# maybeLx/MVSFormerPlusPlus

Hardware: NVIDIA H100
Metric: depth-maps/sec (hot path: FMT + 4-stage cascade) (higher is better)
Workload: dtype f32

## Files before the change

### include/mvsf_b200.h

```cpp
#ifndef MVSF_B200_H
#define MVSF_B200_H

#include <stddef.h>
#include <stdint.h>

#ifdef __cplusplus
extern "C" {
#endif

typedef void* mvsf_stream_t;

enum mvsf_status {
  MVSF_OK = 0,
  MVSF_ERR_INVALID = -1,
  MVSF_ERR_CUDA = -2,
  MVSF_ERR_WORKSPACE = -3
};

const char* mvsf_last_error(void);
int mvsf_abi_version(void);
long long mvsf_launch_count(int reset);
int mvsf_ktimer_enable(int on);
int mvsf_ktimer_read(const char* name, double* ms, long long* launches);

// ... 1 lines not shown
int mvsf_nhwc_to_nchw(const float* src, float* dst, int N, int C, int HW, mvsf_stream_t stream);

int mvsf_compose_geometry(const float* proj, int V, float* homs, float* kinv_ref, mvsf_stream_t stream);

int mvsf_homography_from_proj(const float* src_proj, const float* ref_proj, int B, float* homs, mvsf_stream_t stream);

int mvsf_init_inverse_range(const float* depth_values, int Dn, float* out, int D, int H, int W, mvsf_stream_t stream);
int mvsf_schedule_inverse_range(const float* prev_depth, const float* prev_hypo, int Dp, float split_itv, float* out,
                                int D, int H, int W, mvsf_stream_t stream);
int mvsf_position3d(const float* kinv_ref, const float* depth, const float* depth_values, int Dn, float* stats,
                    int compute_minmax, float* pos, int D, int H, int W, mvsf_stream_t stream);

int mvsf_homo_warp(const float* src_nhwc, const float* hom, const float* depth, float* warped, uint8_t* mask, int C,
                   int D, int H, int W, mvsf_stream_t stream);

int mvsf_warp_corr_set_tile_path(int mode);
int mvsf_warp_corr_set_max_window_miss(int permille);
int mvsf_warp_corr_last_selection(int* used_pipeline, int* miss_permille);

int mvsf_set_prefer_shared_carveout(int on);

int mvsf_warp_corr_plan(int C, int G, int D, int H, int W, int V, size_t spill_budget_bytes);

int mvsf_warp_corr_entropy(const float* feat, const float* homs, const float* depth, float* entropy, int V, int C,
                           int G, int D, int H, int W, mvsf_stream_t stream);
int mvsf_vis_cnn_set_precision(int x_lo);

int mvsf_vis_cnn(const float* entropy, const float* wts, float* vis, int N, int H, int W, mvsf_stream_t stream);
int mvsf_warp_corr_aggregate(const float* feat, const float* homs, const float* depth, const float* vis,
                             float* volume, int V, int C, int G, int D, int H, int W, mvsf_stream_t stream);
int mvsf_warp_corr_entropy_store(const float* feat, const float* homs, const float* depth, float* entropy, float* corr,
                                 int V, int C, int G, int D, int H, int W, mvsf_stream_t stream);
int mvsf_corr_aggregate(const float* corr, const float* vis, float* volume, int V, int G, int D, int H, int W,
                        mvsf_stream_t stream);

int mvsf_costreg_unet_workspace_bytes(int kind, int C, int D, int H, int W, size_t* bytes);
int mvsf_costreg_unet_tc_bytes(size_t* bytes);
int mvsf_costreg_unet_pack_tc(int kind, const float* wts, void* wts_tc, size_t wts_tc_bytes, mvsf_stream_t stream);
int mvsf_costreg_unet_forward(int kind, const float* volume, const float* wts, const void* wts_tc, float* logits,
                              void* workspace, size_t workspace_bytes, int C, int D, int H, int W, mvsf_stream_t stream);
int mvsf_conv3d_tc_layer(int mode, int sd, const float* in, const float* w32, const float* skip, float* out,
                         void* workspace, size_t workspace_bytes, int cin, int cout, int ID, int IH, int IW,
                         mvsf_stream_t stream);

int mvsf_costreg_tr_workspace_bytes(int C, int D, int H, int W, size_t* bytes);
int mvsf_costreg_tr_forward(float* volume, const float* pos, const float* wts, const void* wts16, size_t n_wts,
                            float* logits, void* workspace, size_t workspace_bytes, int C, int D, int H, int W,
                            int layers, float softmax_scale, mvsf_stream_t stream);
int mvsf_split_weights_f16(const float* wts, void* out16, size_t n, mvsf_stream_t stream);

int mvsf_attention_forward(const float* qkv, float* out, void* workspace, size_t workspace_bytes, int N,
                           float softmax_scale, mvsf_stream_t stream);

int mvsf_linear_tc_forward(const float* A, const float* W, const float* bias, float* C, void* workspace,
                           size_t workspace_bytes, int M, int N, int K, int gelu, mvsf_stream_t stream);
int mvsf_linear_tc_epilogue(int epi, const float* A, int lda, const float* W, const float* bias, const float* res,
                            int ldres, const float* gamma, const float* ln_w, const float* ln_b, float ln_eps,
                            int elu_cols, float* C, int ldc, float* Cpre, int ldcpre, void* C2, int ldc2,
                            void* workspace, size_t workspace_bytes, int M, int N, int K, mvsf_stream_t stream);
int mvsf_linear_tc_streamed_epilogue(int epi, const float* A, int lda, const float* W, const float* bias,
                                     const float* res, int ldres, const float* gamma, int elu_cols, float* C, int ldc,
                                     void* C2, int ldc2, void* workspace, size_t workspace_bytes, int M, int N, int K,
                                     mvsf_stream_t stream);

int mvsf_softargmax(const float* logits, const float* depth_hypo, float tmp, float* prob, float* depth, float* conf,
                    int D, int H, int W, mvsf_stream_t stream);
int mvsf_conf_accumulate(const float* conf, int h, int w, float* acc, int H, int W, float scale, int init,
                         mvsf_stream_t stream);

int mvsf_fmt_workspace_bytes(int V, int H1, int W1, size_t* bytes);
int mvsf_fmt_forward(const float* f1, const float* f2, const float* f3, const float* f4, const float* pe,
                     const float* wts, const void* wts16, size_t n_wts, float* o1, float* o2, float* o3, float* o4,
                     void* workspace, size_t workspace_bytes, int V, int H1, int W1, mvsf_stream_t stream);

int mvsf_fpn_encoder_workspace_bytes(int N, int H, int W, size_t* bytes);
int mvsf_fpn_encoder_forward(const float* x, const float* wts, const void* wts_tc, float* c01, float* c11, float* c21,
                             float* c31, void* workspace, size_t workspace_bytes, int N, int H, int W, mvsf_stream_t stream);
int mvsf_fpn_encoder_vit_forward(const float* x, const float* vit_feat, int V, const float* wts, const void* wts_tc,
                                 float* c01, float* c11, float* c21, float* c31, void* workspace, size_t workspace_bytes,
                                 int N, int H, int W, mvsf_stream_t stream);
int mvsf_fpn_decoder_workspace_bytes(int N, int H, int W, size_t* bytes);
int mvsf_fpn_decoder_forward(const float* c01, const float* c11, const float* c21, const float* c31, const float* wts,
                             const void* wts_tc, float* o0, float* o1, float* o2, float* o3, void* workspace,
                             size_t workspace_bytes, int N, int H, int W, mvsf_stream_t stream);
int mvsf_fpn_tc_bytes(int part, size_t* bytes);
int mvsf_fpn_pack_tc(int part, const float* wts, void* wts_tc, size_t wts_tc_bytes, mvsf_stream_t stream);

int mvsf_vit_decoder_workspace_bytes(int B, int V, int h, int w, size_t* bytes);
int mvsf_vit_decoder_tc_bytes(size_t* bytes);
int mvsf_vit_decoder_pack_tc(const float* wts, void* wts_tc, size_t wts_tc_bytes, mvsf_stream_t stream);
int mvsf_vit_decoder_forward(const float* x0, const float* x1, const float* x2, const float* wts, const void* wts_tc,
                             float* out, void* workspace, size_t workspace_bytes, int B, int V, int h, int w,
                             mvsf_stream_t stream);

int mvsf_vit_workspace_bytes(int n, int gh, int gw, size_t* bytes);
int mvsf_vit_tc_bytes(size_t* bytes);
int mvsf_vit_pack_tc(const float* wts, void* wts_tc, size_t wts_tc_bytes, mvsf_stream_t stream);
int mvsf_vit_forward(const float* img, const float* pos, const float* wts, const void* wts_tc, float* out0, float* out1,
                     float* out2, void* workspace, size_t workspace_bytes, int n, int gh, int gw, mvsf_stream_t stream);
int mvsf_vit_forward_image(const float* img, int H, int W, const float* pos, const float* wts, const void* wts_tc,
                           float* out0, float* out1, float* out2, void* workspace, size_t workspace_bytes, int n, int gh,
                           int gw, mvsf_stream_t stream);
int mvsf_vit_attention_forward(const float* qkv, int ldq, float* out, int ldo, void* workspace, size_t workspace_bytes,
                               int n, int N, mvsf_stream_t stream);

#ifdef __cplusplus
// ... 4 lines not shown
```

### mvsformerplusplus_b200/_lib.py

```python
import ctypes
import os

_HERE = os.path.dirname(os.path.abspath(__file__))
LIB_PATH = os.environ.get("MVSF_LIB_PATH") or os.path.join(_HERE, "libmvsf_b200.so")
_lib = None

P, I, F, Z = ctypes.c_void_p, ctypes.c_int, ctypes.c_float, ctypes.c_size_t
SIGNATURES = {
    "mvsf_abi_version": ([], I),
    "mvsf_launch_count": ([I], ctypes.c_longlong),
    "mvsf_ktimer_enable": ([I], I),
    "mvsf_ktimer_read": ([ctypes.c_char_p, ctypes.POINTER(ctypes.c_double), ctypes.POINTER(ctypes.c_longlong)], I),
    "mvsf_nchw_to_nhwc": ([P, P, I, I, I, P], I),
    "mvsf_nhwc_to_nchw": ([P, P, I, I, I, P], I),
    "mvsf_compose_geometry": ([P, I, P, P, P], I),
    "mvsf_homography_from_proj": ([P, P, I, P, P], I),
    "mvsf_init_inverse_range": ([P, I, P, I, I, I, P], I),
    "mvsf_schedule_inverse_range": ([P, P, I, F, P, I, I, I, P], I),
    "mvsf_position3d": ([P, P, P, I, P, I, P, I, I, I, P], I),
    "mvsf_homo_warp": ([P, P, P, P, P, I, I, I, I, P], I),
    "mvsf_warp_corr_set_tile_path": ([I], I),
    "mvsf_warp_corr_set_max_window_miss": ([I], I),
    "mvsf_set_prefer_shared_carveout": ([I], I),
    "mvsf_warp_corr_last_selection": ([ctypes.POINTER(I), ctypes.POINTER(I)], I),
    "mvsf_warp_corr_plan": ([I, I, I, I, I, I, Z], I),
    "mvsf_warp_corr_entropy": ([P, P, P, P, I, I, I, I, I, I, P], I),
    "mvsf_vis_cnn_set_precision": ([I], I),
    "mvsf_vis_cnn": ([P, P, P, I, I, I, P], I),
    "mvsf_warp_corr_aggregate": ([P, P, P, P, P, I, I, I, I, I, I, P], I),
    "mvsf_warp_corr_entropy_store": ([P, P, P, P, P, I, I, I, I, I, I, P], I),
    "mvsf_corr_aggregate": ([P, P, P, I, I, I, I, I, P], I),
    "mvsf_costreg_unet_workspace_bytes": ([I, I, I, I, I, ctypes.POINTER(Z)], I),
    "mvsf_costreg_unet_tc_bytes": ([ctypes.POINTER(Z)], I),
    "mvsf_costreg_unet_pack_tc": ([I, P, P, Z, P], I),
    "mvsf_costreg_unet_forward": ([I, P, P, P, P, P, Z, I, I, I, I, P], I),
    "mvsf_conv3d_tc_layer": ([I, I, P, P, P, P, P, Z, I, I, I, I, I, P], I),
    "mvsf_costreg_tr_workspace_bytes": ([I, I, I, I, ctypes.POINTER(Z)], I),
    "mvsf_costreg_tr_forward": ([P, P, P, P, Z, P, P, Z, I, I, I, I, I, F, P], I),
    "mvsf_split_weights_f16": ([P, P, Z, P], I),
    "mvsf_attention_forward": ([P, P, P, Z, I, F, P], I),
    "mvsf_linear_tc_forward": ([P, P, P, P, P, Z, I, I, I, I, P], I),
    "mvsf_linear_tc_epilogue": ([I, P, I, P, P, P, I, P, P, P, F, I, P, I, P, I, P, I, P, Z, I, I, I, P], I),
    "mvsf_softargmax": ([P, P, F, P, P, P, I, I, I, P], I),
    "mvsf_conf_accumulate": ([P, I, I, P, I, I, F, I, P], I),
    "mvsf_fmt_workspace_bytes": ([I, I, I, ctypes.POINTER(Z)], I),
    "mvsf_fmt_forward": ([P] * 7 + [Z] + [P] * 5 + [Z, I, I, I, P], I),
    "mvsf_fpn_encoder_workspace_bytes": ([I, I, I, ctypes.POINTER(Z)], I),
    "mvsf_fpn_encoder_forward": ([P] * 8 + [Z, I, I, I, P], I),
    "mvsf_fpn_encoder_vit_forward": ([P, P, I] + [P] * 7 + [Z, I, I, I, P], I),
    "mvsf_fpn_decoder_workspace_bytes": ([I, I, I, ctypes.POINTER(Z)], I),
    "mvsf_fpn_decoder_forward": ([P] * 11 + [Z, I, I, I, P], I),
    "mvsf_fpn_tc_bytes": ([I, ctypes.POINTER(Z)], I),
    "mvsf_fpn_pack_tc": ([I, P, P, Z, P], I),
    "mvsf_linear_tc_streamed_epilogue": ([I, P, I, P, P, P, I, P, I, P, I, P, I, P, Z, I, I, I, P], I),
    "mvsf_vit_decoder_workspace_bytes": ([I, I, I, I, ctypes.POINTER(Z)], I),
    "mvsf_vit_decoder_tc_bytes": ([ctypes.POINTER(Z)], I),
    "mvsf_vit_decoder_pack_tc": ([P, P, Z, P], I),
    "mvsf_vit_decoder_forward": ([P] * 7 + [Z, I, I, I, I, P], I),
    "mvsf_vit_workspace_bytes": ([I, I, I, ctypes.POINTER(Z)], I),
    "mvsf_vit_tc_bytes": ([ctypes.POINTER(Z)], I),
    "mvsf_vit_pack_tc": ([P, P, Z, P], I),
    "mvsf_vit_forward": ([P] * 8 + [Z, I, I, I, P], I),
    "mvsf_vit_forward_image": ([P, I, I] + [P] * 7 + [Z, I, I, I, P], I),
    "mvsf_vit_attention_forward": ([P, I, P, I, P, Z, I, I, P], I),
}


def lib():
    global _lib
    if _lib is None:
        if not os.path.exists(LIB_PATH):
            raise RuntimeError(f"{LIB_PATH} is missing: build it with `python -m mvsformerplusplus_b200.build` "
                               "(the hot path has no CPU/PyTorch fallback)")
        L = ctypes.CDLL(LIB_PATH)
        L.mvsf_last_error.restype = ctypes.c_char_p
        L.mvsf_last_error.argtypes = []
        for name, (argt, rest) in SIGNATURES.items():
            fn = getattr(L, name)
            fn.argtypes = argt
            fn.restype = rest
        if os.environ.get("MVSF_VIS_XLO") in ("0", "1"):
            L.mvsf_vis_cnn_set_precision(int(os.environ["MVSF_VIS_XLO"]))
        if os.environ.get("MVSF_WARP_TILE", "1") in ("0", "2"):
            L.mvsf_warp_corr_set_tile_path(int(os.environ["MVSF_WARP_TILE"]))
        if os.environ.get("MVSF_PREFER_SHARED") in ("0", "1"):
            L.mvsf_set_prefer_shared_carveout(int(os.environ["MVSF_PREFER_SHARED"]))
        if os.environ.get("MVSF_WT_MAX_MISS"):
            L.mvsf_warp_corr_set_max_window_miss(int(os.environ["MVSF_WT_MAX_MISS"]))
        _lib = L
    return _lib


def check(rc, what):
    if rc != 0:
        msg = lib().mvsf_last_error().decode(errors="replace")
        raise RuntimeError(f"{what} failed (status {rc}): {msg}")


def launch_count(reset=False):
    return int(lib().mvsf_launch_count(1 if reset else 0))


class profile_calls:

    def __init__(self):
        self.records = []

    def __enter__(self):
        import torch
        L = lib()
        self._orig = {}
        for name in SIGNATURES:
            if name.endswith("_workspace_bytes") or name in ("mvsf_abi_version", "mvsf_launch_count", "mvsf_ktimer_enable",
                                                             "mvsf_ktimer_read", "mvsf_warp_corr_plan",
                                                             "mvsf_warp_corr_set_tile_path", "mvsf_warp_corr_set_max_window_miss", "mvsf_set_prefer_shared_carveout",
                                                             "mvsf_warp_corr_last_selection", "mvsf_vis_cnn_set_precision"):
                continue
            fn = getattr(L, name)
            self._orig[name] = fn

            def wrapped(*a, _fn=fn, _name=name):
                s, e = torch.cuda.Event(enable_timing=True), torch.cuda.Event(enable_timing=True)
                s.record()
                rc = _fn(*a)
                e.record()
                self.records.append((_name, s, e))
                return rc
            setattr(L, name, wrapped)
        return self

    def __exit__(self, *exc):
        L = lib()
        for name, fn in self._orig.items():
            setattr(L, name, fn)
        return False

    def summary(self):
        import torch
        torch.cuda.synchronize()
        out = {}
        for name, s, e in self.records:
            d = out.setdefault(name, {"ms": 0.0, "calls": 0})
            d["ms"] += s.elapsed_time(e)
            d["calls"] += 1
        return out


def ktimer_enable(on):
    check(lib().mvsf_ktimer_enable(1 if on else 0), "ktimer_enable")


def ktimer_read(name):
    ms, n = ctypes.c_double(0.0), ctypes.c_longlong(0)
    check(lib().mvsf_ktimer_read(name.encode(), ctypes.byref(ms), ctypes.byref(n)), "ktimer_read")
    return ms.value, n.value
```

### mvsformerplusplus_b200/csrc/attention_fa.cuh

```cuda
#pragma once
#include <cuda_fp16.h>

#include "linear_tc.cuh"
#include "softmax_attention.cuh"
#include "wgmma.cuh"

namespace mvsf {

__global__ void qkv_tile_kernel(const float* __restrict__ qkv, __half* __restrict__ tiled, int N, int ntiles, float qscale) {
  const int i = blockIdx.x * blockDim.x + threadIdx.x;
  const int total = ntiles * 128 * 3 * 4 * 2;
  if (i >= total) return;
  const int oct = i & 1, h = (i >> 1) & 3, which = (i >> 3) % 3, tok = i / 24;
  const size_t plane = (size_t)4 * ntiles * 2048;
  const int tile = tok >> 7, r = tok & 127;
  float v[8];
  if (tok < N) {
    const float4 a = ldg4(qkv + (size_t)tok * 192 + which * 64 + h * 16 + oct * 8);
    const float4 b = ldg4(qkv + (size_t)tok * 192 + which * 64 + h * 16 + oct * 8 + 4);
    v[0] = a.x; v[1] = a.y; v[2] = a.z; v[3] = a.w; v[4] = b.x; v[5] = b.y; v[6] = b.z; v[7] = b.w;
    if (which == 0) {
#pragma unroll
      for (int e = 0; e < 8; ++e) v[e] *= qscale;
    }
  } else {
#pragma unroll
    for (int e = 0; e < 8; ++e) v[e] = 0.f;
  }
  if (which < 2) {
    __half* ph = tiled + (size_t)(which * 2) * plane + ((size_t)h * ntiles + tile) * 2048;
    __half* pl = ph + plane;
    split_store8(ph + oct * 1024 + r * 8, pl + oct * 1024 + r * 8, v);
  } else {
    __half* pv = tiled + (size_t)4 * plane + ((size_t)h * ntiles + tile) * 5120;
    const int kc = r >> 3, e = r & 7;
#pragma unroll
    for (int d = 0; d < 8; ++d) {
      __half hi, lo;
      gmma::split_f16(v[d], hi, lo);
      pv[kc * 320 + (oct * 8 + d) * 8 + e] = lo;
      pv[kc * 320 + (16 + oct * 8 + d) * 8 + e] = hi;
    }
    if (oct == 0) {
      pv[kc * 320 + 32 * 8 + e] = __float2half_rn(1.0f);
    } else {
#pragma unroll
      for (int z = 33; z < 40; ++z) pv[kc * 320 + z * 8 + e] = __float2half_rn(0.f);
    }
  }
}

namespace fa {
using namespace gmma;
template <int NWG_>
struct Layout {
  static constexpr int NWG = NWG_, NKV = 3, REGS_PRODUCER = 32, REGS_CONSUMER = 160, HD = 16, NH = 4, O_REGS = 20;
  static constexpr uint32_t LBO_QK = 2048, LBO_Q = 1024, LBO_V = 640;
  static constexpr uint32_t K_TILE = 4096, Q_BLOCK = 4096, V_TILE = 16 * LBO_V;
  static constexpr uint32_t OFF_K = 0, OFF_V = OFF_K + NKV * 2 * K_TILE, OFF_Q = OFF_V + NKV * V_TILE,
                            OFF_BAR = OFF_Q + NWG * Q_BLOCK, SMEM = OFF_BAR + 8 + 32 * NKV;
  static constexpr int THREADS = 128 * (NWG + 1);

  const __half* tiled;
  const __half* base;
  size_t plane, head_tiles;

  struct QOperand { uint64_t hi, lo; };
  static __device__ __forceinline__ QOperand q_operand(uint32_t q) {
    return {make_desc(q, LBO_Q, 128), make_desc(q + Q_BLOCK / 2, LBO_Q, 128)};
  }
  static __device__ __forceinline__ void issue_scores(float (&S)[64], const QOperand& q, uint32_t kt) {
    const uint64_t k_hi = make_desc(kt, LBO_QK, 128), k_lo = make_desc(kt + K_TILE, LBO_QK, 128);
    mma_ss<128>(S, q.lo, k_hi, 0u);
    mma_ss<128>(S, q.hi, k_lo, 1u);
    mma_ss<128>(S, q.hi, k_hi, 1u);
    wg_commit();
  }
  static __device__ __forceinline__ void issue_pv(float (&O)[20], const uint32_t (&ph)[8][4], uint32_t vt) {
#pragma unroll
    for (int i = 0; i < 8; ++i) mma_rs_n40(O, ph[i], make_desc(vt + 2 * i * LBO_V, LBO_V, 128), i > 0 ? 1u : 0u);
    wg_commit();
  }
  static __device__ __forceinline__ void fold_tile(float (&o)[2][4], float (&l)[2], const float (&O)[20], const float (&corr)[2],
                                                   int lane) {
#pragma unroll
    for (int h = 0; h < 2; ++h) {
#pragma unroll
      for (int b = 0; b < 2; ++b)
#pragma unroll
        for (int e = 0; e < 2; ++e) o[h][2 * b + e] = fmaf(o[h][2 * b + e], corr[h], O[4 * b + 2 * h + e] + O[4 * (b + 2) + 2 * h + e]);
      const float lt = __shfl_sync(0xffffffffu, O[16 + 2 * h], lane & ~3);
      l[h] = fmaf(l[h], corr[h], lt);
    }
  }
  static __device__ __forceinline__ int q_blocks(int N, int ntiles) { return 2 * ntiles; }
  __device__ __forceinline__ void load_q(uint32_t dst, int b, uint32_t bar) const {
    for (int p = 0; p < 2; ++p)
      for (int kc = 0; kc < 2; ++kc)
        bulk_load(dst + p * (Q_BLOCK / 2) + kc * LBO_Q, base + p * plane + (size_t)(b >> 1) * 2048 + kc * 1024 + (b & 1) * 512,
                  LBO_Q, bar);
  }
  __device__ __forceinline__ const __half* k_tile(int t, int p) const { return base + (2 + p) * plane + (size_t)t * 2048; }
  __device__ __forceinline__ const __half* v_tile(int t) const { return tiled + 4 * plane + (head_tiles + t) * (V_TILE / 2); }
  __device__ __forceinline__ size_t row(int t) const { return (size_t)t; }
};
}

template <int NWG>
__global__ void __launch_bounds__(fa::Layout<NWG>::THREADS, 1)
attention_fa_kernel(const __half* __restrict__ tiled, float* __restrict__ out, __half* __restrict__ out2, int N, int ntiles) {
  const int head = blockIdx.y;
  const size_t head_tiles = (size_t)head * ntiles;
  const fa::Layout<NWG> lay{tiled, tiled + head_tiles * 2048, (size_t)4 * ntiles * 2048, head_tiles};
  attn::softmax_attention(lay, out, 64, out2, N, ntiles);
}

}
```

### mvsformerplusplus_b200/csrc/costreg_tr.cu

```cuda
#include <cuda_fp16.h>
#include <float.h>

#include "attention_fa.cuh"
#include "linear_tc.cuh"
#include "wgmma.cuh"

namespace mvsf {

constexpr int TR_PE = 0, TR_DOWN_W = 192, TR_DOWN_B = TR_DOWN_W + 64 * 256, TR_DOWN_LNW = TR_DOWN_B + 64,
              TR_DOWN_LNB = TR_DOWN_LNW + 64, TR_LAYER0 = TR_DOWN_LNB + 64;
constexpr int L_QKV = 0, L_PROJ_W = 192 * 64, L_PROJ_B = L_PROJ_W + 64 * 64, L_G1 = L_PROJ_B + 64, L_N1W = L_G1 + 64,
              L_N1B = L_N1W + 64, L_F1W = L_N1B + 64, L_F1B = L_F1W + 256 * 64, L_F2W = L_F1B + 256,
              L_F2B = L_F2W + 64 * 256, L_G2 = L_F2B + 64, L_N2W = L_G2 + 64, L_N2B = L_N2W + 64, TR_LAYER = L_N2B + 64;
constexpr int U_W = 0, U_B = 256 * 64, U_LNW = U_B + 256, U_LNB = U_LNW + 8, U_PW = U_LNB + 8, U_PB = U_PW + 8;

__global__ void pe3d_add_kernel(float* __restrict__ vol, const float* __restrict__ pos, const float* __restrict__ pe_w,
                                size_t nvox) {
  __shared__ float w[8 * 24];
  for (int i = threadIdx.x; i < 192; i += blockDim.x) w[i] = __ldg(pe_w + i);
  __syncthreads();
  size_t i = (size_t)blockIdx.x * blockDim.x + threadIdx.x;
  if (i >= nvox) return;
  const float div[4] = {1.0f, 0.1f, 0.01f, 0.001f};
  float pe[24];
// ... 18 lines not shown
    o[c] += s;
  }
  v[0] = make_float4(o[0], o[1], o[2], o[3]);
  v[1] = make_float4(o[4], o[5], o[6], o[7]);
}

__global__ void patch_gather_kernel(const float* __restrict__ vol, __half* __restrict__ patches2, int D, int H, int W) {
  const int Hp = H / 4, Wp = W / 4;
  size_t total = (size_t)(D / 2) * Hp * Wp * 32;
  size_t i = (size_t)blockIdx.x * blockDim.x + threadIdx.x;
  if (i >= total) return;
  int vox = (int)(i & 31);
  size_t t = i >> 5;
  int wp = (int)(t % Wp), hp = (int)((t / Wp) % Hp), dp = (int)(t / ((size_t)Wp * Hp));
  int kw = vox & 3, kh = (vox >> 2) & 3, kd = vox >> 4;
  const float* src = vol + (((size_t)(dp * 2 + kd) * H + hp * 4 + kh) * W + wp * 4 + kw) * 8;
  float4 a = ldg4(src), b = ldg4(src + 4);
  float v[8] = {a.x, a.y, a.z, a.w, b.x, b.y, b.z, b.w};
  __half* row = patches2 + t * 512 + vox * 8;
  split_store8(row, row + 256, v);
}

__global__ void unpatch_ln_prob_kernel(const float* __restrict__ u, const float* __restrict__ tail,
                                       float* __restrict__ logits, int D, int H, int W) {
  const int Hp = H / 4, Wp = W / 4;
  size_t total = (size_t)D * H * W;
  size_t i = (size_t)blockIdx.x * blockDim.x + threadIdx.x;
  if (i >= total) return;
  int vox = (int)(i & 31);
  size_t t = i >> 5;
  int wp = (int)(t % Wp), hp = (int)((t / Wp) % Hp), dp = (int)(t / ((size_t)Wp * Hp));
  int kw = vox & 3, kh = (vox >> 2) & 3, kd = vox >> 4;
  float4 a = ldg4(u + i * 8), b = ldg4(u + i * 8 + 4);
  float x[8] = {a.x, a.y, a.z, a.w, b.x, b.y, b.z, b.w};
  float mean = 0.f;
#pragma unroll
  for (int c = 0; c < 8; ++c) mean += x[c];
  mean *= 0.125f;
  float var = 0.f;
#pragma unroll
  for (int c = 0; c < 8; ++c) { float dd = x[c] - mean; var = fmaf(dd, dd, var); }
  var *= 0.125f;
  const float sd = sqrtf(var + 1e-6f);
  float s = __ldg(tail + (U_PB - U_LNW));
#pragma unroll
  for (int c = 0; c < 8; ++c) {
    float y = __ldg(tail + c) * __fdiv_rn(x[c] - mean, sd) + __ldg(tail + 8 + c);
    s = fmaf(y, __ldg(tail + 16 + c), s);
  }
  logits[((size_t)(dp * 2 + kd) * H + hp * 4 + kh) * W + wp * 4 + kw] = s;
}


static int run_attention(const float* qkv, float* o, __half* o2, __half* tiled, int N, float scale_log2e, cudaStream_t s) {
  constexpr int NWG = 3;
  using A = fa::Layout<NWG>;
  const int ntiles = cdiv(N, 128);
  qkv_tile_kernel<<<cdiv((long long)ntiles * 128 * 24, 256), 256, 0, s>>>(qkv, tiled, N, ntiles, scale_log2e);
  MVSF_LAUNCH_CHECK("qkv_tile");
  static DeviceOnce once;
  const int dev = current_device();
  if (once.need(dev)) {
    MVSF_CUDA_OK(cudaFuncSetAttribute(attention_fa_kernel<NWG>, cudaFuncAttributeMaxDynamicSharedMemorySize, (int)A::SMEM));
    once.done(dev);
  }
  cudaEvent_t kt = ktimer_enabled() ? ktimer_begin("attention_tc", s) : nullptr;
  attention_fa_kernel<NWG><<<dim3(cdiv(N, 64 * NWG), 4), A::THREADS, A::SMEM, s>>>(tiled, o, o2, N, ntiles);
  if (kt) ktimer_end(kt, s);
  MVSF_LAUNCH_CHECK("attention_tc");
  return MVSF_OK;
}

}

using namespace mvsf;

extern "C" {

int mvsf_costreg_tr_workspace_bytes(int C, int D, int H, int W, size_t* bytes) {
  MVSF_REQUIRE(bytes && C == 8, "costreg_tr: base channel must be 8");
  MVSF_REQUIRE(D % 2 == 0 && H % 4 == 0 && W % 4 == 0 && D > 0 && H > 0 && W > 0,
               "costreg_tr: D %% 2, H %% 4, W %% 4 must be 0 (down_rate (2,4,4))");
  size_t N = (size_t)(D / 2) * (H / 4) * (W / 4);
  *bytes = (N * (256 + 64 + 64 + 64 + 64 + 64 + 192) + (N + 128) * 224) * sizeof(float);
  return MVSF_OK;
}

int mvsf_costreg_tr_forward(float* volume, const float* pos, const float* wts, const void* wts16, size_t n_wts,
                            float* logits, void* workspace, size_t workspace_bytes, int C, int D, int H, int W,
                            int layers, float softmax_scale, mvsf_stream_t stream) {
  MVSF_REQUIRE(volume && wts && wts16 && logits && workspace && layers >= 0, "costreg_tr: bad arguments");
  size_t need = 0;
  int rc = mvsf_costreg_tr_workspace_bytes(C, D, H, W, &need);
  if (rc) return rc;
  if (workspace_bytes < need) return fail(MVSF_ERR_WORKSPACE, "costreg_tr: workspace %zu < %zu bytes", workspace_bytes, need);
  MVSF_REQUIRE(((uintptr_t)workspace & 15) == 0 && ((uintptr_t)wts & 15) == 0 && ((uintptr_t)volume & 15) == 0 &&
                   ((uintptr_t)wts16 & 15) == 0 && (n_wts % 8) == 0,
               "costreg_tr: pointers must be 16-byte aligned");
  MVSF_REQUIRE(n_wts >= (size_t)TR_LAYER0 + (size_t)layers * TR_LAYER + U_PB + 1, "costreg_tr: weight blob too small");
  cudaStream_t s = (cudaStream_t)stream;
  const size_t nvox = (size_t)D * H * W;
  const int N = (int)((size_t)(D / 2) * (H / 4) * (W / 4));
  const __half* wh = reinterpret_cast<const __half*>(wts16);
  const __half* wl = wh + n_wts;
  float* big = (float*)workspace;
  __half* big2 = reinterpret_cast<__half*>(big);
  float* x = big + (size_t)N * 256;
  float* y = x + (size_t)N * 64;
  __half* x2 = reinterpret_cast<__half*>(y + (size_t)N * 64);
  __half* y2 = x2 + (size_t)N * 128;
  __half* o2 = y2 + (size_t)N * 128;
  float* qkv = reinterpret_cast<float*>(o2 + (size_t)N * 128);
  __half* split = reinterpret_cast<__half*>(qkv + (size_t)N * 192);

  if (pos) {
    pe3d_add_kernel<<<cdiv((long long)nvox, 256), 256, 0, s>>>(volume, pos, wts + TR_PE, nvox);
    MVSF_LAUNCH_CHECK("pe3d_add");
  }
  patch_gather_kernel<<<cdiv((long long)N * 32, 256), 256, 0, s>>>(volume, big2, D, H, W);
  MVSF_LAUNCH_CHECK("patch_gather");

  TcLinArgs a{};
  a.Ah = big2; a.Al = big2 + 256; a.lda = 512; a.Bh = wh + TR_DOWN_W; a.Bl = wl + TR_DOWN_W; a.ldb = 256;
  a.M = N; a.N = 64; a.K = 256; a.bias = wts + TR_DOWN_B; a.ln_w = wts + TR_DOWN_LNW; a.ln_b = wts + TR_DOWN_LNB; a.ln_eps = 1e-6f;
  a.C = x; a.ldc = 64; a.C2 = x2; a.ldc2 = 128;
  if ((rc = launch_linear_tc(a, LIN_LN, s))) return rc;

  const float scale_log2e = softmax_scale * 1.4426950408889634f;
  for (int l = 0; l < layers; ++l) {
    const size_t lo = (size_t)TR_LAYER0 + (size_t)l * TR_LAYER;
    const float* lw = wts + lo;
    TcLinArgs q{};
    q.Ah = x2; q.Al = x2 + 64; q.lda = 128; q.Bh = wh + lo + L_QKV; q.Bl = wl + lo + L_QKV; q.ldb = 64;
    q.M = N; q.N = 192; q.K = 64; q.C = qkv; q.ldc = 192;
    if ((rc = launch_linear_tc(q, LIN_BIAS, s))) return rc;
    if ((rc = run_attention(qkv, nullptr, o2, split, N, scale_log2e, s))) return rc;
    TcLinArgs p{};
    p.Ah = o2; p.Al = o2 + 64; p.lda = 128; p.Bh = wh + lo + L_PROJ_W; p.Bl = wl + lo + L_PROJ_W; p.ldb = 64;
    p.M = N; p.N = 64; p.K = 64; p.bias = lw + L_PROJ_B; p.res = x; p.ldres = 64; p.gamma = lw + L_G1;
    p.ln_w = lw + L_N1W; p.ln_b = lw + L_N1B; p.ln_eps = 1e-5f; p.C = y; p.ldc = 64; p.C2 = y2; p.ldc2 = 128;
    if ((rc = launch_linear_tc(p, LIN_RES_LN, s))) return rc;
    TcLinArgs f1{};
    f1.Ah = y2; f1.Al = y2 + 64; f1.lda = 128; f1.Bh = wh + lo + L_F1W; f1.Bl = wl + lo + L_F1W; f1.ldb = 64;
    f1.M = N; f1.N = 256; f1.K = 64; f1.bias = lw + L_F1B; f1.C2 = big2; f1.ldc2 = 512;
    if ((rc = launch_linear_tc(f1, LIN_GELU, s))) return rc;
    TcLinArgs f2{};
    f2.Ah = big2; f2.Al = big2 + 256; f2.lda = 512; f2.Bh = wh + lo + L_F2W; f2.Bl = wl + lo + L_F2W; f2.ldb = 256;
    f2.M = N; f2.N = 64; f2.K = 256; f2.bias = lw + L_F2B; f2.res = y; f2.ldres = 64; f2.gamma = lw + L_G2;
    f2.ln_w = lw + L_N2W; f2.ln_b = lw + L_N2B; f2.ln_eps = 1e-5f; f2.C = x; f2.ldc = 64; f2.C2 = x2; f2.ldc2 = 128;
    if ((rc = launch_linear_tc(f2, LIN_RES_LN, s))) return rc;
  }
  const size_t uo = (size_t)TR_LAYER0 + (size_t)layers * TR_LAYER;
  TcLinArgs u{};
  u.Ah = x2; u.Al = x2 + 64; u.lda = 128; u.Bh = wh + uo + U_W; u.Bl = wl + uo + U_W; u.ldb = 64;
  u.M = N; u.N = 256; u.K = 64; u.bias = wts + uo + U_B; u.C = big; u.ldc = 256;
  if ((rc = launch_linear_tc(u, LIN_BIAS, s))) return rc;
  unpatch_ln_prob_kernel<<<cdiv((long long)nvox, 256), 256, 0, s>>>(big, wts + uo + U_LNW, logits, D, H, W);
  MVSF_LAUNCH_CHECK("unpatch_ln_prob");
  return MVSF_OK;
}

int mvsf_attention_forward(const float* qkv, float* out, void* workspace, size_t workspace_bytes, int N,
                           float softmax_scale, mvsf_stream_t stream) {
  MVSF_REQUIRE(qkv && out && workspace && N > 0, "attention_forward: bad arguments");
  if (workspace_bytes < (size_t)(N + 128) * 896) return fail(MVSF_ERR_WORKSPACE, "attention_forward: workspace %zu < %zu bytes", workspace_bytes, (size_t)(N + 128) * 896);
  return run_attention(qkv, out, nullptr, reinterpret_cast<__half*>(workspace), N, softmax_scale * 1.4426950408889634f, (cudaStream_t)stream);
}
}
```

### mvsformerplusplus_b200/csrc/softmax_attention.cuh

```cuda
#pragma once
#include <cuda_fp16.h>

#include "wgmma.cuh"

namespace mvsf {
namespace attn {
using namespace gmma;

__device__ __forceinline__ void softmax_tile(float (&S)[64], float (&m)[2], float (&corr)[2], int j, int N, int q) {
  if (j * 128 + 128 > N) {
#pragma unroll
    for (int i = 0; i < 64; ++i)
      if (j * 128 + 8 * (i >> 2) + 2 * q + (i & 1) >= N) S[i] = -1e30f;
  }
  float mb[2];
#pragma unroll
  for (int h = 0; h < 2; ++h) {
    float pmax = -1e30f;
#pragma unroll
    for (int b = 0; b < 16; ++b) pmax = fmaxf(pmax, fmaxf(S[4 * b + 2 * h], S[4 * b + 2 * h + 1]));
    pmax = fmaxf(pmax, __shfl_xor_sync(0xffffffffu, pmax, 1));
    pmax = fmaxf(pmax, __shfl_xor_sync(0xffffffffu, pmax, 2));
    const float mx = fmaxf(m[h], pmax);
    corr[h] = ex2f(m[h] - mx);
    m[h] = mx;
    mb[h] = mx - 14.0f;
  }
#pragma unroll
  for (int i = 0; i < 64; ++i) S[i] = ex2f(S[i] - mb[(i >> 1) & 1]);
}
__device__ __forceinline__ void pack_p(const float (&S)[64], uint32_t (&ph)[8][4]) {
#pragma unroll
  for (int i = 0; i < 8; ++i)
#pragma unroll
    for (int r = 0; r < 4; ++r) ph[i][r] = pack_half2(S[8 * i + 2 * r], S[8 * i + 2 * r + 1]);
}

template <class L>
__device__ __forceinline__ void softmax_attention(const L& lay, float* __restrict__ out, int ldo, __half* __restrict__ out2,
                                                  int N, int ntiles) {
  constexpr int NWG = L::NWG, NKV = L::NKV;
  static_assert(128 * (L::REGS_PRODUCER + NWG * L::REGS_CONSUMER) <= 65536, "setmaxnreg exceeds the register file");
  extern __shared__ __align__(128) unsigned char smem[];
  const int tid = threadIdx.x, warp = tid >> 5, lane = tid & 31;
  const int head = blockIdx.y;
  const uint32_t sb = smem_u32(smem);
  const uint32_t bar_q = sb + L::OFF_BAR, bar_kf = bar_q + 8, bar_ke = bar_kf + 8 * NKV, bar_vf = bar_ke + 8 * NKV,
                 bar_ve = bar_vf + 8 * NKV;
  if (tid == 0) {
    mbar_init(bar_q, 1);
    for (int i = 0; i < NKV; ++i) { mbar_init(bar_kf + 8 * i, 1); mbar_init(bar_ke + 8 * i, NWG); mbar_init(bar_vf + 8 * i, 1); mbar_init(bar_ve + 8 * i, NWG); }
    fence_barrier_init();
  }
  __syncthreads();

  if (warp >= 4 * NWG) {
    asm volatile("setmaxnreg.dec.sync.aligned.u32 %0;" ::"n"(L::REGS_PRODUCER));
    if (warp == 4 * NWG && lane == 0) {
      const int nqb = L::q_blocks(N, ntiles);
      expect_tx(bar_q, NWG * L::Q_BLOCK);
      for (int w = 0; w < NWG; ++w) lay.load_q(sb + L::OFF_Q + w * L::Q_BLOCK, min(NWG * (int)blockIdx.x + w, nqb - 1), bar_q);
      for (int t = 0; t < ntiles; ++t) {
        const int s = t % NKV;
        const uint32_t par = (uint32_t)(((t / NKV) & 1) ^ 1);
        mbar_wait(bar_ke + 8 * s, par);
        expect_tx(bar_kf + 8 * s, 2 * L::K_TILE);
        bulk_load(sb + L::OFF_K + (2 * s) * L::K_TILE, lay.k_tile(t, 0), L::K_TILE, bar_kf + 8 * s);
        bulk_load(sb + L::OFF_K + (2 * s + 1) * L::K_TILE, lay.k_tile(t, 1), L::K_TILE, bar_kf + 8 * s);
        mbar_wait(bar_ve + 8 * s, par);
        expect_tx(bar_vf + 8 * s, L::V_TILE);
        bulk_load(sb + L::OFF_V + s * L::V_TILE, lay.v_tile(t), L::V_TILE, bar_vf + 8 * s);
      }
    }
    return;
  }
  asm volatile("setmaxnreg.inc.sync.aligned.u32 %0;" ::"n"(L::REGS_CONSUMER));
  const int wg = warp >> 2, wq = warp & 3, q = lane & 3;
  const bool leader = (tid & 127) == 0;
  const typename L::QOperand qs = L::q_operand(sb + L::OFF_Q + wg * L::Q_BLOCK);
  float o[2][L::HD / 4];
  float m[2] = {-1e30f, -1e30f}, l[2] = {0.f, 0.f};
#pragma unroll
  for (int h = 0; h < 2; ++h)
#pragma unroll
    for (int d = 0; d < L::HD / 4; ++d) o[h][d] = 0.f;
  float S[64], O[L::O_REGS], corr[2];
  uint32_t ph[8][4];
  mbar_wait(bar_q, 0u);
  mbar_wait(bar_kf, 0u);
  wg_fence();
  L::issue_scores(S, qs, sb + L::OFF_K);
  wg_wait<0>();
  fence_regs<64>(S);
  if (leader) mbar_arrive(bar_ke);
  softmax_tile(S, m, corr, 0, N, q);
  pack_p(S, ph);
  if (ntiles > 1) {
    mbar_wait(bar_kf + 8, 0u);
    mbar_wait(bar_vf, 0u);
  }
  for (int j = 0; j + 1 < ntiles; ++j) {
    const int s = j % NKV, s1 = (j + 1) % NKV, s2 = (j + 2) % NKV;
    wg_fence();
    L::issue_scores(S, qs, sb + L::OFF_K + (2 * s1) * L::K_TILE);
    L::issue_pv(O, ph, sb + L::OFF_V + s * L::V_TILE);
    wg_wait<1>();
    fence_regs<64>(S);
    if (leader) mbar_arrive(bar_ke + 8 * s1);
    float corr1[2];
    softmax_tile(S, m, corr1, j + 1, N, q);
    if (j + 2 < ntiles) mbar_wait(bar_kf + 8 * s2, (uint32_t)(((j + 2) / NKV) & 1));
    mbar_wait(bar_vf + 8 * s1, (uint32_t)(((j + 1) / NKV) & 1));
    wg_wait<0>();
    fence_regs<L::O_REGS>(O);
    if (leader) mbar_arrive(bar_ve + 8 * s);
    L::fold_tile(o, l, O, corr, lane);
    pack_p(S, ph);
    corr[0] = corr1[0];
    corr[1] = corr1[1];
  }
  {
    const int j = ntiles - 1, s = j % NKV;
    mbar_wait(bar_vf + 8 * s, (uint32_t)((j / NKV) & 1));
    wg_fence();
    L::issue_pv(O, ph, sb + L::OFF_V + s * L::V_TILE);
    wg_wait<0>();
    fence_regs<L::O_REGS>(O);
    L::fold_tile(o, l, O, corr, lane);
  }
  constexpr int W = L::NH * L::HD;
#pragma unroll
  for (int h = 0; h < 2; ++h) {
    const int t = 64 * (NWG * (int)blockIdx.x + wg) + 16 * wq + (lane >> 2) + 8 * h;
    if (t >= N) continue;
    const size_t r = lay.row(t);
    const float inv = __fdiv_rn(1.0f, l[h]);
#pragma unroll
    for (int b = 0; b < L::HD / 8; ++b) {
      const int col = head * L::HD + 8 * b + 2 * q;
      const float r0 = o[h][2 * b] * inv, r1 = o[h][2 * b + 1] * inv;
      if (out) *reinterpret_cast<float2*>(out + r * ldo + col) = make_float2(r0, r1);
      if (out2) split_store2(out2 + r * (2 * W) + col, out2 + r * (2 * W) + W + col, r0, r1);
    }
  }
}

}
}
```

### mvsformerplusplus_b200/csrc/vit_attention.cuh

```cuda
#pragma once
#include <cuda_fp16.h>

#include "linear_tc.cuh"
#include "softmax_attention.cuh"
#include "wgmma.cuh"

namespace mvsf {
namespace vfa {
using namespace gmma;
constexpr int NH = 12, HD = 64;
constexpr uint32_t LBO_K = 2048, LBO_Q = 1024;
constexpr uint32_t K_TILE = 8 * LBO_K;
constexpr uint32_t Q_TILE = 8 * LBO_Q;
constexpr int VROWS = 136;
constexpr uint32_t LBO_V = VROWS * 16, V_TILE = 16 * LBO_V, V_LO = 9 * 128;
__host__ __device__ constexpr size_t q_plane(int nqb) { return (size_t)nqb * (Q_TILE / 2); }
__host__ __device__ constexpr size_t k_plane(int nt) { return (size_t)nt * (K_TILE / 2); }
__host__ __device__ constexpr size_t v_plane(int nt) { return (size_t)nt * (V_TILE / 2); }
__host__ __device__ constexpr size_t tiled_halves(int n, int nt) {
  return (size_t)n * NH * (2 * q_plane(2 * nt) + 2 * k_plane(nt) + v_plane(nt));
}

__host__ __device__ __forceinline__ size_t token_row(int b, int t, int n, int N, bool cls_last) {
  if (!cls_last) return (size_t)b * N + t;
// ... 5 lines not shown
                                    int nt, bool cls_last, float qscale) {
  using namespace vfa;
  const long long i = (long long)blockIdx.x * blockDim.x + threadIdx.x;
  const long long total = (long long)n * nt * 128 * 3 * NH * 8;
  if (i >= total) return;
  const int oct = (int)(i & 7), head = (int)((i >> 3) % NH), which = (int)((i / (8 * NH)) % 3);
  const long long bt = i / (8 * NH * 3);
  const int t = (int)(bt % (nt * 128)), b = (int)(bt / (nt * 128));
  float v[8];
  if (t < N) {
    const float* src = qkv + token_row(b, t, n, N, cls_last) * ldq + which * (NH * HD) + head * HD + oct * 8;
    const float4 a = ldg4(src), c = ldg4(src + 4);
    v[0] = a.x; v[1] = a.y; v[2] = a.z; v[3] = a.w; v[4] = c.x; v[5] = c.y; v[6] = c.z; v[7] = c.w;
    if (which == 0) {
#pragma unroll
      for (int e = 0; e < 8; ++e) v[e] *= qscale;
    }
  } else {
#pragma unroll
    for (int e = 0; e < 8; ++e) v[e] = 0.f;
  }
  const size_t bh = (size_t)b * NH + head, qp = q_plane(2 * nt), kp = k_plane(nt);
  const size_t planes = (size_t)n * NH;
  if (which == 0) {
    __half* ph = tiled + bh * qp + (size_t)(t >> 6) * (Q_TILE / 2) + oct * (LBO_Q / 2) + (t & 63) * 8;
    split_store8(ph, ph + planes * qp, v);
  } else if (which == 1) {
    __half* ph = tiled + 2 * planes * qp + bh * kp + (size_t)(t >> 7) * (K_TILE / 2) + oct * (LBO_K / 2) + (t & 127) * 8;
    split_store8(ph, ph + planes * kp, v);
  } else {
    __half* pv = tiled + 2 * planes * (qp + kp) + bh * v_plane(nt) + (size_t)(t >> 7) * (V_TILE / 2) +
                 ((t & 127) >> 3) * (LBO_V / 2) + (t & 7);
#pragma unroll
    for (int d = 0; d < 8; ++d) {
      const __half hi = __float2half_rn(v[d]);
      pv[(oct * 8 + d) * 8] = hi;
      pv[(72 + oct * 8 + d) * 8] = __float2half_rn(v[d] - __half2float(hi));
    }
    if (oct == 0) pv[64 * 8] = __float2half_rn(t < N ? 1.0f : 0.0f);
    if (oct == 1) {
#pragma unroll
      for (int z = 65; z < 72; ++z) pv[z * 8] = __float2half_rn(0.f);
    }
  }
}

namespace vfa {
struct Layout {
  static constexpr int NWG = 2, NKV = 2, REGS_PRODUCER = 40, REGS_CONSUMER = 232, HD = vfa::HD, NH = vfa::NH, O_REGS = 36;
  static constexpr uint32_t K_TILE = vfa::K_TILE, V_TILE = vfa::V_TILE, Q_BLOCK = 2 * Q_TILE;
  static constexpr uint32_t OFF_K = 0, OFF_V = OFF_K + NKV * 2 * K_TILE, OFF_Q = OFF_V + NKV * V_TILE,
                            OFF_BAR = OFF_Q + NWG * Q_BLOCK, SMEM = OFF_BAR + 8 + 32 * NKV;
  static constexpr int THREADS = 128 * (NWG + 1);

  const __half* qbase;
  const __half* kbase;
  const __half* vbase;
  size_t planes, qp, kp;
  int img, n, N;
  bool cls_last;

  using QOperand = uint32_t;
  static __device__ __forceinline__ QOperand q_operand(uint32_t q) { return q; }
  static __device__ __forceinline__ void issue_scores(float (&S)[64], uint32_t q, uint32_t kt) {
#pragma unroll
    for (int i = 0; i < 4; ++i)
      mma_ss<128>(S, make_desc(q + Q_TILE + 2 * i * LBO_Q, LBO_Q, 128), make_desc(kt + 2 * i * LBO_K, LBO_K, 128),
                  i > 0 ? 1u : 0u);
#pragma unroll
    for (int i = 0; i < 4; ++i)
      mma_ss<128>(S, make_desc(q + 2 * i * LBO_Q, LBO_Q, 128), make_desc(kt + K_TILE + 2 * i * LBO_K, LBO_K, 128), 1u);
#pragma unroll
    for (int i = 0; i < 4; ++i)
      mma_ss<128>(S, make_desc(q + 2 * i * LBO_Q, LBO_Q, 128), make_desc(kt + 2 * i * LBO_K, LBO_K, 128), 1u);
    wg_commit();
  }
  static __device__ __forceinline__ void issue_pv(float (&O)[36], const uint32_t (&ph)[8][4], uint32_t vt) {
#pragma unroll
    for (int i = 0; i < 8; ++i) mma_rs_n72(O, ph[i], make_desc(vt + 2 * i * LBO_V, LBO_V, 128), i > 0 ? 1u : 0u);
#pragma unroll
    for (int i = 0; i < 8; ++i) mma_rs_n64(O, ph[i], make_desc(vt + 2 * i * LBO_V + V_LO, LBO_V, 128), 1u);
    wg_commit();
  }
  static __device__ __forceinline__ void fold_tile(float (&o)[2][16], float (&l)[2], const float (&O)[36], const float (&corr)[2],
                                                   int lane) {
#pragma unroll
    for (int h = 0; h < 2; ++h) {
#pragma unroll
      for (int b = 0; b < 8; ++b)
#pragma unroll
        for (int e = 0; e < 2; ++e) o[h][2 * b + e] = fmaf(o[h][2 * b + e], corr[h], O[4 * b + 2 * h + e]);
      const float lt = __shfl_sync(0xffffffffu, O[32 + 2 * h], lane & ~3);
      l[h] = fmaf(l[h], corr[h], lt);
    }
  }
  static __device__ __forceinline__ int q_blocks(int N, int nt) { return (N + 63) / 64; }
  __device__ __forceinline__ void load_q(uint32_t dst, int b, uint32_t bar) const {
    for (int p = 0; p < 2; ++p) bulk_load(dst + p * Q_TILE, qbase + p * planes * qp + (size_t)b * (Q_TILE / 2), Q_TILE, bar);
  }
  __device__ __forceinline__ const __half* k_tile(int t, int p) const { return kbase + p * planes * kp + (size_t)t * (K_TILE / 2); }
  __device__ __forceinline__ const __half* v_tile(int t) const { return vbase + (size_t)t * (V_TILE / 2); }
  __device__ __forceinline__ size_t row(int t) const { return token_row(img, t, n, N, cls_last); }
};
}

__global__ void __launch_bounds__(vfa::Layout::THREADS, 1)
// ... 13 lines not shown
```

Baseline: 45.76.

## Split tail attention work items across KV ranges with a merge kernel

Reworks the cost-regularization transformer attention launch into a 1D list of work items. The leftover tail items (items modulo SM count) are split across KV tile ranges, so idle SMs in the last wave get work. Each split item writes partial outputs with the running max and sum into workspace after the tile planes. A small merge kernel then rescales and combines the partials. The aim is less wave-quantization idle time, paid for with an extra launch, partial write/read traffic, and workspace-size dependence.

```diff
diff --git a/include/mvsf_b200.h b/include/mvsf_b200.h
--- a/include/mvsf_b200.h
+++ b/include/mvsf_b200.h
@@ -77,6 +77,8 @@
 int mvsf_attention_forward(const float* qkv, float* out, void* workspace, size_t workspace_bytes, int N,
                            float softmax_scale, mvsf_stream_t stream);
 
+int mvsf_attention_split_plan(int N, int num_sms, int* split_items, int* parts);
+
 int mvsf_linear_tc_forward(const float* A, const float* W, const float* bias, float* C, void* workspace,
                            size_t workspace_bytes, int M, int N, int K, int gelu, mvsf_stream_t stream);
 int mvsf_linear_tc_epilogue(int epi, const float* A, int lda, const float* W, const float* bias, const float* res,
diff --git a/mvsformerplusplus_b200/_lib.py b/mvsformerplusplus_b200/_lib.py
--- a/mvsformerplusplus_b200/_lib.py
+++ b/mvsformerplusplus_b200/_lib.py
@@ -39,6 +39,7 @@
     "mvsf_costreg_tr_forward": ([P, P, P, P, Z, P, P, Z, I, I, I, I, I, F, P], I),
     "mvsf_split_weights_f16": ([P, P, Z, P], I),
     "mvsf_attention_forward": ([P, P, P, Z, I, F, P], I),
+    "mvsf_attention_split_plan": ([I, I, ctypes.POINTER(I), ctypes.POINTER(I)], I),
     "mvsf_linear_tc_forward": ([P, P, P, P, P, Z, I, I, I, I, P], I),
     "mvsf_linear_tc_epilogue": ([I, P, I, P, P, P, I, P, P, P, F, I, P, I, P, I, P, I, P, Z, I, I, I, P], I),
     "mvsf_softargmax": ([P, P, F, P, P, P, I, I, I, P], I),
@@ -112,7 +113,7 @@
         self._orig = {}
         for name in SIGNATURES:
             if name.endswith("_workspace_bytes") or name in ("mvsf_abi_version", "mvsf_launch_count", "mvsf_ktimer_enable",
-                                                             "mvsf_ktimer_read", "mvsf_warp_corr_plan",
+                                                             "mvsf_ktimer_read", "mvsf_warp_corr_plan", "mvsf_attention_split_plan",
                                                              "mvsf_warp_corr_set_tile_path", "mvsf_warp_corr_set_max_window_miss", "mvsf_set_prefer_shared_carveout",
                                                              "mvsf_warp_corr_last_selection", "mvsf_vis_cnn_set_precision"):
                 continue
diff --git a/mvsformerplusplus_b200/csrc/attention_fa.cuh b/mvsformerplusplus_b200/csrc/attention_fa.cuh
--- a/mvsformerplusplus_b200/csrc/attention_fa.cuh
+++ b/mvsformerplusplus_b200/csrc/attention_fa.cuh
@@ -1,5 +1,7 @@
 #pragma once
 #include <cuda_fp16.h>
+
+#include <algorithm>
 
 #include "linear_tc.cuh"
 #include "softmax_attention.cuh"
@@ -60,10 +62,14 @@
   static constexpr uint32_t OFF_K = 0, OFF_V = OFF_K + NKV * 2 * K_TILE, OFF_Q = OFF_V + NKV * V_TILE,
                             OFF_BAR = OFF_Q + NWG * Q_BLOCK, SMEM = OFF_BAR + 8 + 32 * NKV;
   static constexpr int THREADS = 128 * (NWG + 1);
+  static constexpr bool SPLIT = true;
+  static constexpr int ROWS = 64 * NWG, PART_FLOATS = ROWS * (HD + 2);
 
   const __half* tiled;
   const __half* base;
   size_t plane, head_tiles;
+  int head, group, t0, t1;
+  float* part;
 
   struct QOperand { uint64_t hi, lo; };
   static __device__ __forceinline__ QOperand q_operand(uint32_t q) {
@@ -106,13 +112,74 @@
 };
 }
 
+namespace fa {
+constexpr size_t TILE_BYTES = (4 * 4 * 2048 + 4 * 5120) * sizeof(__half);
+constexpr int MIN_PART_TILES = 16;
+
+struct SplitPlan { int items, split, parts; };
+template <int NWG>
+inline SplitPlan split_plan(int N, int sms, size_t region_bytes) {
+  using A = Layout<NWG>;
+  const int ntiles = (N + 127) / 128, items = 4 * ((N + A::ROWS - 1) / A::ROWS), r = items % sms;
+  const size_t planes = (size_t)ntiles * TILE_BYTES;
+  const size_t slots = region_bytes > planes ? (region_bytes - planes) / (A::PART_FLOATS * sizeof(float)) : 0;
+  const int k = r ? (int)std::min({(size_t)(sms / r), slots / r, (size_t)(ntiles / MIN_PART_TILES)}) : 0;
+  return k >= 2 ? SplitPlan{items, r, k} : SplitPlan{items, 0, 1};
+}
+}
+
 template <int NWG>
 __global__ void __launch_bounds__(fa::Layout<NWG>::THREADS, 1)
-attention_fa_kernel(const __half* __restrict__ tiled, float* __restrict__ out, __half* __restrict__ out2, int N, int ntiles) {
-  const int head = blockIdx.y;
+attention_fa_kernel(const __half* __restrict__ tiled, float* __restrict__ out, __half* __restrict__ out2, int N, int ntiles,
+                    int split, int parts, float* __restrict__ partials) {
+  using A = fa::Layout<NWG>;
+  const int groups = (N + A::ROWS - 1) / A::ROWS, whole = 4 * groups - split;
+  int item = blockIdx.x, t0 = 0, t1 = ntiles;
+  float* part = nullptr;
+  if (item >= whole) {
+    const int b = item - whole, p = b % parts;
+    item = whole + b / parts;
+    t0 = p * ntiles / parts;
+    t1 = (p + 1) * ntiles / parts;
+    part = partials + (size_t)b * A::PART_FLOATS;
+  }
+  const int head = item / groups;
   const size_t head_tiles = (size_t)head * ntiles;
-  const fa::Layout<NWG> lay{tiled, tiled + head_tiles * 2048, (size_t)4 * ntiles * 2048, head_tiles};
+  const A lay{tiled, tiled + head_tiles * 2048, (size_t)4 * ntiles * 2048, head_tiles, head, item % groups, t0, t1, part};
   attn::softmax_attention(lay, out, 64, out2, N, ntiles);
 }
 
+template <int NWG>
+__global__ void attention_merge_kernel(const float* __restrict__ partials, float* __restrict__ out, __half* __restrict__ out2,
+                                       int N, int split, int parts) {
+  using A = fa::Layout<NWG>;
+  constexpr int HD = A::HD, W = A::NH * A::HD, ROWS = A::ROWS;
+  const int i = blockIdx.x * blockDim.x + threadIdx.x;
+  if (i >= split * ROWS) return;
+  const int groups = (N + ROWS - 1) / ROWS, s = i / ROWS, rr = i % ROWS, item = 4 * groups - split + s;
+  const int head = item / groups, t = (item % groups) * ROWS + rr;
+  if (t >= N) return;
+  const float* p0 = partials + (size_t)s * parts * A::PART_FLOATS + (size_t)rr * (HD + 2);
+  float mx = -1e30f;
+  for (int p = 0; p < parts; ++p) mx = fmaxf(mx, p0[(size_t)p * A::PART_FLOATS + HD]);
+  float o[HD], l = 0.f;
+#pragma unroll
+  for (int d = 0; d < HD; ++d) o[d] = 0.f;
+  for (int p = 0; p < parts; ++p) {
+    const float* pp = p0 + (size_t)p * A::PART_FLOATS;
+    const float w = gmma::ex2f(pp[HD] - mx);
+    l = fmaf(pp[HD + 1], w, l);
+#pragma unroll
+    for (int d = 0; d < HD; ++d) o[d] = fmaf(pp[d], w, o[d]);
+  }
+  const float inv = __fdiv_rn(1.0f, l);
+#pragma unroll
+  for (int d = 0; d < HD; d += 2) {
+    const int col = head * HD + d;
+    const float r0 = o[d] * inv, r1 = o[d + 1] * inv;
+    if (out) *reinterpret_cast<float2*>(out + (size_t)t * W + col) = make_float2(r0, r1);
+    if (out2) gmma::split_store2(out2 + (size_t)t * (2 * W) + col, out2 + (size_t)t * (2 * W) + W + col, r0, r1);
+  }
 }
+
+}
diff --git a/mvsformerplusplus_b200/csrc/costreg_tr.cu b/mvsformerplusplus_b200/csrc/costreg_tr.cu
--- a/mvsformerplusplus_b200/csrc/costreg_tr.cu
+++ b/mvsformerplusplus_b200/csrc/costreg_tr.cu
@@ -94,8 +94,11 @@
 }
 
 
+constexpr int ATT_NWG = 3;
+static size_t attention_workspace_bytes(int N) { return (size_t)(N + 128) * 896; }
+
 static int run_attention(const float* qkv, float* o, __half* o2, __half* tiled, int N, float scale_log2e, cudaStream_t s) {
-  constexpr int NWG = 3;
+  constexpr int NWG = ATT_NWG;
   using A = fa::Layout<NWG>;
   const int ntiles = cdiv(N, 128);
   qkv_tile_kernel<<<cdiv((long long)ntiles * 128 * 24, 256), 256, 0, s>>>(qkv, tiled, N, ntiles, scale_log2e);
@@ -106,10 +109,18 @@
     MVSF_CUDA_OK(cudaFuncSetAttribute(attention_fa_kernel<NWG>, cudaFuncAttributeMaxDynamicSharedMemorySize, (int)A::SMEM));
     once.done(dev);
   }
+  const fa::SplitPlan plan = fa::split_plan<NWG>(N, device_sm_count(dev), attention_workspace_bytes(N));
+  float* partials = reinterpret_cast<float*>(reinterpret_cast<unsigned char*>(tiled) + (size_t)ntiles * fa::TILE_BYTES);
   cudaEvent_t kt = ktimer_enabled() ? ktimer_begin("attention_tc", s) : nullptr;
-  attention_fa_kernel<NWG><<<dim3(cdiv(N, 64 * NWG), 4), A::THREADS, A::SMEM, s>>>(tiled, o, o2, N, ntiles);
+  attention_fa_kernel<NWG><<<plan.items - plan.split + plan.split * plan.parts, A::THREADS, A::SMEM, s>>>(
+      tiled, o, o2, N, ntiles, plan.split, plan.parts, partials);
+  MVSF_LAUNCH_CHECK("attention_tc");
+  if (plan.split) {
+    attention_merge_kernel<NWG><<<cdiv((long long)plan.split * A::ROWS, 128), 128, 0, s>>>(partials, o, o2, N, plan.split,
+                                                                                            plan.parts);
+    MVSF_LAUNCH_CHECK("attention_merge");
+  }
   if (kt) ktimer_end(kt, s);
-  MVSF_LAUNCH_CHECK("attention_tc");
   return MVSF_OK;
 }
 
@@ -205,7 +216,15 @@
 int mvsf_attention_forward(const float* qkv, float* out, void* workspace, size_t workspace_bytes, int N,
                            float softmax_scale, mvsf_stream_t stream) {
   MVSF_REQUIRE(qkv && out && workspace && N > 0, "attention_forward: bad arguments");
-  if (workspace_bytes < (size_t)(N + 128) * 896) return fail(MVSF_ERR_WORKSPACE, "attention_forward: workspace %zu < %zu bytes", workspace_bytes, (size_t)(N + 128) * 896);
+  if (workspace_bytes < attention_workspace_bytes(N)) return fail(MVSF_ERR_WORKSPACE, "attention_forward: workspace %zu < %zu bytes", workspace_bytes, attention_workspace_bytes(N));
   return run_attention(qkv, out, nullptr, reinterpret_cast<__half*>(workspace), N, softmax_scale * 1.4426950408889634f, (cudaStream_t)stream);
 }
-}
+
+int mvsf_attention_split_plan(int N, int num_sms, int* split_items, int* parts) {
+  MVSF_REQUIRE(N > 0 && num_sms > 0 && split_items && parts, "attention_split_plan: bad arguments");
+  const fa::SplitPlan p = fa::split_plan<ATT_NWG>(N, num_sms, attention_workspace_bytes(N));
+  *split_items = p.split;
+  *parts = p.parts;
+  return MVSF_OK;
+}
+}
diff --git a/mvsformerplusplus_b200/csrc/softmax_attention.cuh b/mvsformerplusplus_b200/csrc/softmax_attention.cuh
--- a/mvsformerplusplus_b200/csrc/softmax_attention.cuh
+++ b/mvsformerplusplus_b200/csrc/softmax_attention.cuh
@@ -37,13 +37,27 @@
 }
 
 template <class L>
+__device__ __forceinline__ int item_head(const L& lay) {
+  if constexpr (L::SPLIT) return lay.head; else return blockIdx.y;
+}
+template <class L>
+__device__ __forceinline__ int item_group(const L& lay) {
+  if constexpr (L::SPLIT) return lay.group; else return blockIdx.x;
+}
+
+template <class L>
 __device__ __forceinline__ void softmax_attention(const L& lay, float* __restrict__ out, int ldo, __half* __restrict__ out2,
                                                   int N, int ntiles) {
   constexpr int NWG = L::NWG, NKV = L::NKV;
   static_assert(128 * (L::REGS_PRODUCER + NWG * L::REGS_CONSUMER) <= 65536, "setmaxnreg exceeds the register file");
   extern __shared__ __align__(128) unsigned char smem[];
   const int tid = threadIdx.x, warp = tid >> 5, lane = tid & 31;
-  const int head = blockIdx.y;
+  const int head = item_head(lay);
+  int t0 = 0, nt = ntiles;
+  float* part = nullptr;
+  if constexpr (L::SPLIT) {
+    t0 = lay.t0; nt = lay.t1 - lay.t0; part = lay.part;
+  }
   const uint32_t sb = smem_u32(smem);
   const uint32_t bar_q = sb + L::OFF_BAR, bar_kf = bar_q + 8, bar_ke = bar_kf + 8 * NKV, bar_vf = bar_ke + 8 * NKV,
                  bar_ve = bar_vf + 8 * NKV;
@@ -59,17 +73,17 @@
     if (warp == 4 * NWG && lane == 0) {
       const int nqb = L::q_blocks(N, ntiles);
       expect_tx(bar_q, NWG * L::Q_BLOCK);
-      for (int w = 0; w < NWG; ++w) lay.load_q(sb + L::OFF_Q + w * L::Q_BLOCK, min(NWG * (int)blockIdx.x + w, nqb - 1), bar_q);
-      for (int t = 0; t < ntiles; ++t) {
+      for (int w = 0; w < NWG; ++w) lay.load_q(sb + L::OFF_Q + w * L::Q_BLOCK, min(NWG * item_group(lay) + w, nqb - 1), bar_q);
+      for (int t = 0; t < nt; ++t) {
         const int s = t % NKV;
         const uint32_t par = (uint32_t)(((t / NKV) & 1) ^ 1);
         mbar_wait(bar_ke + 8 * s, par);
         expect_tx(bar_kf + 8 * s, 2 * L::K_TILE);
-        bulk_load(sb + L::OFF_K + (2 * s) * L::K_TILE, lay.k_tile(t, 0), L::K_TILE, bar_kf + 8 * s);
-        bulk_load(sb + L::OFF_K + (2 * s + 1) * L::K_TILE, lay.k_tile(t, 1), L::K_TILE, bar_kf + 8 * s);
+        bulk_load(sb + L::OFF_K + (2 * s) * L::K_TILE, lay.k_tile(t0 + t, 0), L::K_TILE, bar_kf + 8 * s);
+        bulk_load(sb + L::OFF_K + (2 * s + 1) * L::K_TILE, lay.k_tile(t0 + t, 1), L::K_TILE, bar_kf + 8 * s);
         mbar_wait(bar_ve + 8 * s, par);
         expect_tx(bar_vf + 8 * s, L::V_TILE);
-        bulk_load(sb + L::OFF_V + s * L::V_TILE, lay.v_tile(t), L::V_TILE, bar_vf + 8 * s);
+        bulk_load(sb + L::OFF_V + s * L::V_TILE, lay.v_tile(t0 + t), L::V_TILE, bar_vf + 8 * s);
       }
     }
     return;
@@ -93,13 +107,13 @@
   wg_wait<0>();
   fence_regs<64>(S);
   if (leader) mbar_arrive(bar_ke);
-  softmax_tile(S, m, corr, 0, N, q);
+  softmax_tile(S, m, corr, t0, N, q);
   pack_p(S, ph);
-  if (ntiles > 1) {
+  if (nt > 1) {
     mbar_wait(bar_kf + 8, 0u);
     mbar_wait(bar_vf, 0u);
   }
-  for (int j = 0; j + 1 < ntiles; ++j) {
+  for (int j = 0; j + 1 < nt; ++j) {
     const int s = j % NKV, s1 = (j + 1) % NKV, s2 = (j + 2) % NKV;
     wg_fence();
     L::issue_scores(S, qs, sb + L::OFF_K + (2 * s1) * L::K_TILE);
@@ -108,8 +122,8 @@
     fence_regs<64>(S);
     if (leader) mbar_arrive(bar_ke + 8 * s1);
     float corr1[2];
-    softmax_tile(S, m, corr1, j + 1, N, q);
-    if (j + 2 < ntiles) mbar_wait(bar_kf + 8 * s2, (uint32_t)(((j + 2) / NKV) & 1));
+    softmax_tile(S, m, corr1, t0 + j + 1, N, q);
+    if (j + 2 < nt) mbar_wait(bar_kf + 8 * s2, (uint32_t)(((j + 2) / NKV) & 1));
     mbar_wait(bar_vf + 8 * s1, (uint32_t)(((j + 1) / NKV) & 1));
     wg_wait<0>();
     fence_regs<L::O_REGS>(O);
@@ -120,7 +134,7 @@
     corr[1] = corr1[1];
   }
   {
-    const int j = ntiles - 1, s = j % NKV;
+    const int j = nt - 1, s = j % NKV;
     mbar_wait(bar_vf + 8 * s, (uint32_t)((j / NKV) & 1));
     wg_fence();
     L::issue_pv(O, ph, sb + L::OFF_V + s * L::V_TILE);
@@ -128,10 +142,23 @@
     fence_regs<L::O_REGS>(O);
     L::fold_tile(o, l, O, corr, lane);
   }
+  if constexpr (L::SPLIT) {
+    if (part) {
+#pragma unroll
+      for (int h = 0; h < 2; ++h) {
+        float* pr = part + (size_t)(64 * wg + 16 * wq + (lane >> 2) + 8 * h) * (L::HD + 2);
+#pragma unroll
+        for (int b = 0; b < L::HD / 8; ++b)
+          *reinterpret_cast<float2*>(pr + 8 * b + 2 * q) = make_float2(o[h][2 * b], o[h][2 * b + 1]);
+        if (q == 0) *reinterpret_cast<float2*>(pr + L::HD) = make_float2(m[h], l[h]);
+      }
+      return;
+    }
+  }
   constexpr int W = L::NH * L::HD;
 #pragma unroll
   for (int h = 0; h < 2; ++h) {
-    const int t = 64 * (NWG * (int)blockIdx.x + wg) + 16 * wq + (lane >> 2) + 8 * h;
+    const int t = 64 * (NWG * item_group(lay) + wg) + 16 * wq + (lane >> 2) + 8 * h;
     if (t >= N) continue;
     const size_t r = lay.row(t);
     const float inv = __fdiv_rn(1.0f, l[h]);
diff --git a/mvsformerplusplus_b200/csrc/vit_attention.cuh b/mvsformerplusplus_b200/csrc/vit_attention.cuh
--- a/mvsformerplusplus_b200/csrc/vit_attention.cuh
+++ b/mvsformerplusplus_b200/csrc/vit_attention.cuh
@@ -81,6 +81,7 @@
   static constexpr uint32_t OFF_K = 0, OFF_V = OFF_K + NKV * 2 * K_TILE, OFF_Q = OFF_V + NKV * V_TILE,
                             OFF_BAR = OFF_Q + NWG * Q_BLOCK, SMEM = OFF_BAR + 8 + 32 * NKV;
   static constexpr int THREADS = 128 * (NWG + 1);
+  static constexpr bool SPLIT = false;
 
   const __half* qbase;
   const __half* kbase;
```

After: 47.57, median of 6. 1.04x the previous value.
